# Francesco215/autoregressive_diffusion

Measured on AMD Instinct MI355X. Metric: denoiser-step frames/sec at 1/2/4/8 MI355X; 64-frame Lunar-Lander seq, higher is better.
Workload: dtype bf16; 1 GPU; Lunar-Lander 64-frame seq, gym EDM2 UNet 46.2M (gym_train.py:37-47), 8 seq/GPU (gym_train.py:55 micro_batch_size), step = EDM2Loss fwd + bwd + grad all-reduce + [grad-norm clip +] AdamW + 2 EMA profiles, 3:1 mix of 3-D/2-D steps; global_batch=8, seq_len=64, parallelism=dp1, hip_graph=False

## Files before the change

autoregressive_diffusion_amd/csrc/conv_glds.h:

```cpp
#pragma once
#include <type_traits>
#include "conv_kernels.h"

#include "lds_dma.h"

#ifdef CONV_STAMP
#define CSTAMP_DECL unsigned long long st_t = __builtin_amdgcn_s_memtime(), st_acc[12] = {0, 0, 0, 0, 0, 0, 0, 0, 0, 0, 0, 0};
#define CSTAMP(i) { const unsigned long long n_ = __builtin_amdgcn_s_memtime(); st_acc[i] += n_ - st_t; st_t = n_; }
#define CSTAMP2(c, i, j) { if (c) CSTAMP(i) else CSTAMP(j) }
#else
#define CSTAMP_DECL
#define CSTAMP(i)
#define CSTAMP2(c, i, j)
#endif

template <int NT, int PW, int NW, int MT, int WC = 1>
struct GldsCfg {
  static constexpr int NWP = NW / WC;
  static constexpr int NPOS = 32 * NWP * MT, NTHR = 64 * NW, BN = 32 * NT * WC;
  using P = Patch<PW, NPOS>;
  static constexpr int HW = (PW == 8) ? 12 : PW + 2, HH = P::PH + 2, FT = P::FT;
  static constexpr int HALO = FT * HH * HW;
  static constexpr int SROWS = (HALO + 15) / 16 * 16;
  static constexpr int AROWS = 2 * SROWS, CROWS = HALO, WROWS = 9 * BN;
  static constexpr int BUF = (AROWS + WROWS) * 64;
  static constexpr int EROW = NT * 32 * 2 + 16;
  static constexpr int EPI = NW * 32 * EROW;
  static_assert(PW == 16 || PW == 8, "tile geometries of the LDS-DMA kernel");
  static constexpr int LDS_BYTES = (2 * BUF > EPI) ? 2 * BUF : EPI;
  static_assert(LDS_BYTES <= 160 * 1024, "two staging buffers must fit the 160 KB LDS");
  static constexpr int BUFC = (SROWS + WROWS) * 64;
  static constexpr int RES_EOFF = BUF + 2 * BUFC;
  static constexpr int RES_BYTES = RES_EOFF + 2 * FT * BN * 4 + EPI;
  static_assert(2 * FT * BN * 4 + EPI <= BUF, "the epilogue stages through ONE of the two buffers");
  static_assert((NWP * 2 * HW) % 16 == 0 || MT == 1, "position tiles of a wave must be 16-row aligned apart");
};

template <int NT, int PW, int NW, int MT, int WC = 1, bool CTX = true, bool RES = false>
__global__ __launch_bounds__(64 * NW, (NW >= 8) ? 2 : 1) void conv_glds_kernel(const ConvDev d) {
#if defined(__HIP_DEVICE_COMPILE__)
  using Cfg = GldsCfg<NT, PW, NW, MT, WC>;
  using P = typename Cfg::P;
  constexpr int S = 2, TAPS = 9, CK = 32, KS = CK / 16, HW_ = Cfg::HW, HH_ = Cfg::HH, FT = Cfg::FT, NWP = Cfg::NWP;
  constexpr int NPH = CTX ? 3 : 1;
  constexpr int BN = Cfg::BN, NTHR = Cfg::NTHR, AROWS = Cfg::AROWS, BUF = Cfg::BUF;
  static_assert(!RES || (CTX && FT == 1 && Cfg::RES_BYTES <= 160 * 1024), "resident layout: gated conv, one frame per tile");
  __shared__ __attribute__((aligned(16))) unsigned char smem[RES ? Cfg::RES_BYTES : Cfg::LDS_BYTES];

  const OnirisConvArgs& a = d.a;
  const int tid = threadIdx.x, lane = tid & 63, wave = tid >> 6, r = lane & 31, h = lane >> 5;
  const int wp = wave % NWP, wc = wave / NWP;
  const int H = a.H, W = a.W, T = a.T, Cin = a.Cin, HWp = a.H * a.W;

  const int ntiles = d.ntx * d.nty * d.ntt * a.B * d.ncob;
  int tl, tl_hi, tl_step;
  {
    const int nwg = gridDim.x, xcd = blockIdx.x & 7;
    const int q = ntiles >> 3, rr = ntiles & 7;
    const int lo = (xcd < rr) ? xcd * (q + 1) : rr * (q + 1) + (xcd - rr) * q;
    tl_hi = lo + q + ((xcd < rr) ? 1 : 0);
    tl_step = (nwg - xcd + 7) >> 3;
    tl = lo + (blockIdx.x >> 3);
  }
  if (tl >= tl_hi) return;
  struct Tile { int co0, x0, y0, t0, b; };
  auto decode = [&](int id) __attribute__((always_inline)) {
    Tile t;
    t.co0 = (id % d.ncob) * BN; id /= d.ncob;
    t.x0 = (id % d.ntx) * P::PW; id /= d.ntx;
    t.y0 = (id % d.nty) * P::PH; id /= d.nty;
    t.t0 = (id % d.ntt) * P::FT; id /= d.ntt;
    t.b = id;
    return t;
  };

  int pr = r;
  if constexpr (PW == 16) {
    const bool ga = (r < 4) || (r >= 12 && r < 16) || (r >= 20 && r < 28);
    const int k = ga ? ((r < 4) ? r : (r < 16) ? r - 8 : r - 12) : ((r < 12) ? r - 4 : (r < 20) ? r - 8 : r - 16);
    pr = (ga ? 0 : 16) + k;
  } else {
    const bool ga = (r < 4) || (r >= 12 && r < 16) || (r >= 20 && r < 28);
    const int k = ga ? ((r < 4) ? r : (r < 16) ? r - 8 : r - 12) : ((r < 12) ? r - 4 : (r < 20) ? r - 8 : r - 16);
    pr = ((k >> 3) * 2 + (ga ? 0 : 1)) * 8 + (k & 7);
  }
  int arow[MT];
#pragma unroll
  for (int m = 0; m < MT; ++m) {
    const int p = (wp + NWP * m) * 32 + pr;
    const int ft = p / (P::PH * P::PW), py = (p / P::PW) % P::PH, px = p % P::PW;
    arow[m] = (ft * HH_ + py) * HW_ + px;
  }

  constexpr int TOTA = AROWS * 4, TOTC = Cfg::CROWS * 4, TOTW = Cfg::WROWS * 4;
  constexpr int NIA = (TOTA + NTHR - 1) / NTHR, NIC = (TOTC + NTHR - 1) / NTHR, NIW = (TOTW + NTHR - 1) / NTHR;
  constexpr int OOB = (int)0x80000000;
  const int frame_elems = HWp * Cin;
  int adesc[NIA], wdesc[NIW];
  auto set_adesc = [&](const Tile& t) __attribute__((always_inline)) {
    int tid_ = tid;
    asm volatile("" : "+v"(tid_));
#pragma unroll
    for (int i = 0; i < NIA; ++i) {
      const int e = i * NTHR + tid_;
      const int row = e >> 2, gp = (e & 3) ^ ((row >> 2) & 3);
      const int s = row / Cfg::SROWS, rem = row % Cfg::SROWS;
      const int f_ = rem / (HH_ * HW_), hr = rem % (HH_ * HW_);
      const int y = t.y0 + hr / HW_ - 1, x = t.x0 + hr % HW_ - 1;
      adesc[i] = OOB;
      if (e < TOTA && rem < Cfg::HALO && hr % HW_ < P::PW + 2 && t.t0 + f_ < T && (unsigned)y < (unsigned)H &&
          (unsigned)x < (unsigned)W)
        adesc[i] = ((s * T + f_) * frame_elems + (y * W + x) * Cin + gp * 8) * 2;
    }
  };
#pragma unroll
  for (int i = 0; i < NIW; ++i) {
    const int e = (i * NW + wave) * 64 + lane;
    const int row = e >> 2, gp = (e & 3) ^ ((row >> 2) & 3);
    const int tap = row / BN, co = row % BN;
    wdesc[i] = ((tap * a.CoutP + co) * a.CinP + gp * 8) * 2;
  }
  const int wbytes = TAPS * a.CoutP * a.CinP * 2;
  const i32x4 rs_f = make_rsrc(oniris_fill_rows, 128);
  const i32x4 rs_wo = make_rsrc(a.w_own, wbytes), rs_wc = make_rsrc(CTX ? a.w_ctx : a.w_own, CTX ? 2 * wbytes : wbytes);
  const unsigned lds0 = (unsigned)(size_t)(lds_void_t*)smem;
  const int fillsel = (a.ctx_fill != 0.f) ? 64 : 0;

  auto issue = [&](const Tile& t, int ch, int ph, int bsel) __attribute__((always_inline)) {
    const int c0 = ch * CK;
    const int boff = RES ? ((ph == 0) ? 0 : BUF + (ph - 1) * Cfg::BUFC) : bsel * BUF;
    const int woff = (RES && ph != 0) ? Cfg::SROWS * 64 : AROWS * 64;
    const unsigned dst = __builtin_amdgcn_readfirstlane(lds0 + boff + wave * 1024);
    if (ph == 0) {
      const bf16* xb = (const bf16*)a.x + (size_t)t.b * S * T * frame_elems;
      const i32x4 rs_x = make_rsrc(xb, S * T * frame_elems * 2);
      const int so = (t.t0 * frame_elems + c0) * 2;
#pragma unroll
      for (int i = 0; i < NIA; ++i)
        if ((i * NW + wave) * 64 + lane < TOTA) dma16(rs_x, adesc[i], so, dst + i * NW * 1024);
    } else if constexpr (FT == 1) {
      const int f = t.t0 + ((ph == 1) ? a.coff0 : a.coff1);
      if (f >= 0 && f < a.ctx_T) {
        const bf16* cb_ = (const bf16*)a.ctx + (size_t)t.b * a.ctx_bstride * frame_elems;
        const i32x4 rs_c = make_rsrc(cb_, a.ctx_T * frame_elems * 2);
        const int so = (f * frame_elems + c0) * 2;
#pragma unroll
        for (int i = 0; i < NIC; ++i)
          if ((i * NW + wave) * 64 + lane < TOTC) dma16(rs_c, adesc[i], so, dst + i * NW * 1024);
      } else {
#pragma unroll
        for (int i = 0; i < NIC; ++i)
          if ((i * NW + wave) * 64 + lane < TOTC) dma16(rs_f, (adesc[i] < 0) ? OOB : fillsel, 0, dst + i * NW * 1024);
      }
    } else {
      const int coff = (ph == 1) ? a.coff0 : a.coff1;
      const bf16* cb_ = (const bf16*)a.ctx + (size_t)t.b * a.ctx_bstride * frame_elems;
      const i32x4 rs_c = make_rsrc(cb_, a.ctx_T * frame_elems * 2);
      const int shift = (t.t0 + coff) * frame_elems * 2;
#pragma unroll
      for (int i = 0; i < NIC; ++i) {
        const int e = (i * NW + wave) * 64 + lane;
        if (e < TOTC) {
          const int f = t.t0 + coff + ((e >> 2) % Cfg::SROWS) / (HH_ * HW_);
          if (f >= 0 && f < a.ctx_T) dma16(rs_c, (adesc[i] < 0) ? OOB : adesc[i] + shift, c0 * 2, dst + i * NW * 1024);
          else dma16(rs_f, (adesc[i] < 0) ? OOB : fillsel, 0, dst + i * NW * 1024);
        }
      }
    }
    const int sw = ((t.co0 * a.CinP + c0) + ((ph == 2) ? TAPS * a.CoutP * a.CinP : 0)) * 2;
#ifdef CONV_STAMP
    if (a.big_tile & 64) return;
#endif
    if (ph == 0) {
#pragma unroll
      for (int i = 0; i < NIW; ++i)
        if ((i * NW + wave) * 64 + lane < TOTW) dma16(rs_wo, wdesc[i], sw, dst + woff + i * NW * 1024);
    } else {
#pragma unroll
      for (int i = 0; i < NIW; ++i)
        if ((i * NW + wave) * 64 + lane < TOTW) dma16(rs_wc, wdesc[i], sw, dst + woff + i * NW * 1024);
    }
  };

  const int wa0 = (wc * NT * 32 + r) * 64 + ((h ^ ((r >> 2) & 3)) << 4);
  int xa0[TAPS];
#pragma unroll
  for (int tap = 0; tap < TAPS; ++tap) {
    const int R = arow[0] + (tap / 3) * HW_ + (tap % 3);
    xa0[tap] = R * 64 + ((h ^ ((R >> 2) & 3)) << 4);
  }

  f32x16 acc[S][MT][NT];
  f32x16 accc[MT][NT];

  constexpr int MID_STEP = 4;
  auto mfma_steps = [&](auto own_, int boff, int woff, auto mid) __attribute__((always_inline)) {
    constexpr bool OWN = decltype(own_)::value;
    constexpr int NX = OWN ? S : 1;
    constexpr int NSTEP = TAPS * KS;
    const unsigned char* base = smem + boff;
    const unsigned char* wbase = base + woff;
    bf16x8 wf[2][NT], xf[2][NX][MT];
    auto ld = [&](int fb, int st) __attribute__((always_inline)) {
      const int tap = st / KS, ks = st % KS;
#pragma unroll
      for (int n = 0; n < NT; ++n)
        wf[fb][n] = *(const bf16x8*)(wbase + ((wa0 ^ (ks * 32)) + (tap * BN + n * 32) * 64));
#pragma unroll
      for (int s = 0; s < NX; ++s)
#pragma unroll
        for (int m = 0; m < MT; ++m)
          xf[fb][s][m] = *(const bf16x8*)(base + ((xa0[tap] ^ (ks * 32)) + (s * Cfg::SROWS + m * (NWP * 2 * HW_)) * 64));
    };
    ld(0, 0);
#pragma unroll
    for (int st = 0; st < NSTEP; ++st) {
      mid(st);
      if (st + 1 < NSTEP) ld((st + 1) & 1, st + 1);
#pragma unroll
      for (int m = 0; m < MT; ++m)
#pragma unroll
        for (int n = 0; n < NT; ++n) {
          if constexpr (OWN) {
#pragma unroll
            for (int s = 0; s < S; ++s) acc[s][m][n] = mfma32(wf[st & 1][n], xf[st & 1][s][m], acc[s][m][n]);
          } else {
            accc[m][n] = mfma32(wf[st & 1][n], xf[st & 1][0][m], accc[m][n]);
          }
        }
      if (st + 1 < NSTEP) __builtin_amdgcn_sched_group_barrier(0x100, NT + NX * MT, 0);
      __builtin_amdgcn_sched_group_barrier(0x008, NX * MT * NT, 0);
    }
  };
  auto no_mid = [](int) __attribute__((always_inline)) {};

  constexpr int EROW = Cfg::EROW;
  constexpr int ESC = 2 * FT * BN * 4;
  const int nphase = (Cin / CK) * NPH;
  Tile cur = decode(tl);
  set_adesc(cur);
  int bsel = 0;
  issue(cur, 0, 0, 0);
  if constexpr (RES) { issue(cur, 0, 1, 0); issue(cur, 0, 2, 0); }
  Tile nxt = cur;
  bool more = false;
  int tl_next = tl;
  CSTAMP_DECL
#pragma unroll 1
  for (;;) {
    dma_wait();
    __syncthreads();
    CSTAMP(0)
#pragma unroll
    for (int m = 0; m < MT; ++m)
#pragma unroll
      for (int n = 0; n < NT; ++n) {
#pragma unroll
        for (int i = 0; i < 16; ++i) { acc[0][m][n][i] = 0.f; acc[1][m][n][i] = 0.f; accc[m][n][i] = 0.f; }
      }
    float esc_v = 0.f;
    const int lft = ((wp * 32 + pr) / (P::PH * P::PW)) % FT;
    const bool lvalid = cur.t0 + lft < T;
    const int n0 = (cur.b * S) * T + (lvalid ? cur.t0 + lft : 0), n1 = n0 + T;
    const float cown0 = a.coef_own ? a.coef_own[n0] : 1.f, cown1 = a.coef_own ? a.coef_own[n1] : 1.f;
    const float cctx0 = a.coef_ctx ? a.coef_ctx[n0] : 1.f, cctx1 = a.coef_ctx ? a.coef_ctx[n1] : 1.f;
    if (a.epi == ONIRIS_EPI_EMB_SILU && tid < 2 * FT * BN) {
      const int co = cur.co0 + tid % BN, f_ = (tid / BN) % FT, s_ = tid / (FT * BN);
      if (co < a.Cout && cur.t0 + f_ < T)
        esc_v = ((const float*)a.escale)[(size_t)((cur.b * S + s_) * T + cur.t0 + f_) * (a.escale_pitch ? a.escale_pitch : a.Cout) + co];
    }
    CSTAMP(1)
    if constexpr (!RES) {
#pragma unroll 1
      for (int itp = 0; itp < nphase; ++itp) {
        const int ph = itp % NPH;
        const bool have_next = itp + 1 < nphase;
        const bool early = __builtin_amdgcn_readfirstlane(wave) < NW / 2 || (a.big_tile & 32);
        if (have_next && early) issue(cur, (itp + 1) / NPH, (itp + 1) % NPH, bsel ^ 1);
        auto mid = [&](int st) __attribute__((always_inline)) {
          if (st == MID_STEP && have_next && !early) issue(cur, (itp + 1) / NPH, (itp + 1) % NPH, bsel ^ 1);
        };
        CSTAMP2(ph == 0, 2, 7)
        if (!CTX || ph == 0) mfma_steps(std::true_type{}, bsel * BUF, AROWS * 64, mid);
        else mfma_steps(std::false_type{}, bsel * BUF, AROWS * 64, mid);
#ifdef CONV_STAMP
        asm volatile("" ::"v"(acc[0][0][0]), "v"(acc[1][0][0]), "v"(accc[0][0]), "v"(acc[0][0][NT - 1]), "v"(acc[1][0][NT - 1]), "v"(accc[0][NT - 1]));
#endif
        CSTAMP2(ph == 0, 3, 8)
        dma_wait();
        CSTAMP2(ph == 0, 4, 9)
        __syncthreads();
        CSTAMP2(ph == 0, 5, 10)
        bsel ^= 1;
      }
    }
    unsigned char* stg = smem + (RES ? Cfg::RES_EOFF : (bsel ^ 1) * BUF);
    unsigned char* ep = stg + ESC + wave * 32 * EROW;
    if constexpr (RES) mfma_steps(std::true_type{}, 0, AROWS * 64, no_mid);

    if (a.epi == ONIRIS_EPI_EMB_SILU) {
      if (tid < 2 * FT * BN) *(float*)(stg + tid * 4) = esc_v;
      __syncthreads();
    }
    asm volatile("" ::"v"(cown0), "v"(cown1), "v"(cctx0), "v"(cctx1));
    tl_next = tl + tl_step;
    more = tl_next < tl_hi;
    nxt = cur;
    if constexpr (RES) {
      __syncthreads();
      if (more) { nxt = decode(tl_next); set_adesc(nxt); issue(nxt, 0, 0, 0); }
      mfma_steps(std::false_type{}, BUF, Cfg::SROWS * 64, no_mid);
      __syncthreads();
      if (more) issue(nxt, 0, 1, 0);
      mfma_steps(std::false_type{}, BUF + Cfg::BUFC, Cfg::SROWS * 64, no_mid);
      __syncthreads();
      if (more) issue(nxt, 0, 2, 0);
    } else if (more) {
      nxt = decode(tl_next);
      set_adesc(nxt);
      issue(nxt, 0, 0, bsel);
    }

    bf16* og = (bf16*)a.out;
    bool clip_hit = false;
#pragma unroll
    for (int m = 0; m < MT; ++m) {
      const int ptile = (wp + NWP * m) * 32;
      const int cow = cur.co0 + wc * NT * 32;
      auto flush = [&](bf16* dst, size_t blk) __attribute__((always_inline)) {
        constexpr int PO = NT * 32 / 8;
#pragma unroll
        for (int it = 0; it < 32 * PO / 64; ++it) {
          const int id = it * 64 + lane;
          const int row = id / PO, part = id % PO;
          const int q = ptile + row;
          const int f_ = q / (P::PH * P::PW), yy = (q / P::PW) % P::PH, xx = q % P::PW;
          const size_t px_ = (size_t)(cur.t0 + f_) * HWp + (cur.y0 + yy) * W + (cur.x0 + xx);
          const int co = cow + part * 8;
          if (co < a.Cout && cur.t0 + f_ < T) {
            const u32x4 v_ = *(const u32x4*)(ep + row * EROW + part * 16);
            u32x4* o_ = (u32x4*)(dst + (blk + px_) * a.Cout + co);
            if (d.nt) __builtin_nontemporal_store(v_, o_); else *o_ = v_;
          }
        }
      };
#pragma unroll
      for (int s = 0; s < S; ++s) {
        const float cown = s ? cown1 : cown0, cctx = s ? cctx1 : cctx0;
        const size_t blk = (size_t)(cur.b * S + s) * T * HWp;
        auto raw = [&](int nt, float (&v)[16]) __attribute__((always_inline)) {
#pragma unroll
          for (int i = 0; i < 16; ++i) v[i] = CTX ? __builtin_fmaf(cctx, accc[m][nt][i], cown * acc[s][m][nt][i]) : cown * acc[s][m][nt][i];
        };
        auto put = [&](int nt, const float (&v)[16]) __attribute__((always_inline)) {
#pragma unroll
          for (int g = 0; g < 4; ++g) {
            bf16x4 o;
#pragma unroll
            for (int k = 0; k < 4; ++k) o[k] = f2bf(v[4 * g + k]);
            *(bf16x4*)(ep + pr * EROW + (nt * 32 + 8 * g + 4 * h) * 2) = o;
          }
        };
        float v[16];
        if (a.epi == ONIRIS_EPI_MPSUM) {
          if (a.out2) {
#pragma unroll
            for (int nt = 0; nt < NT; ++nt) { raw(nt, v); put(nt, v); }
            flush((bf16*)a.out2, blk);
          }
          const int p = ptile + pr;
          const size_t obase = (blk + (size_t)(cur.t0 + lft) * HWp + (cur.y0 + (p / P::PW) % P::PH) * W + cur.x0 + p % P::PW) * a.Cout;
#pragma unroll
          for (int nt = 0; nt < NT; ++nt) {
            raw(nt, v);
#pragma unroll
            for (int g = 0; g < 4; ++g) {
              const int co = cow + nt * 32 + 8 * g + 4 * h;
              bf16x4 rv;
#pragma unroll
              for (int k = 0; k < 4; ++k) rv[k] = f2bf(0.f);
              if (co < a.Cout && lvalid) rv = *(const bf16x4*)((const bf16*)a.res + obase + co);
#pragma unroll
              for (int k = 0; k < 4; ++k) {
                float o = a.ta * bf2f(rv[k]) + a.tb * v[4 * g + k];
                if (a.clip > 0.f) {
                  o = fminf(fmaxf(o, -a.clip), a.clip);
                  clip_hit |= !(fabsf(bf2f(f2bf(o))) < a.clip);
                }
                v[4 * g + k] = o;
              }
            }
            put(nt, v);
          }
          flush(og, blk);
        } else {
#pragma unroll
          for (int nt = 0; nt < NT; ++nt) { raw(nt, v); put(nt, v); }
          flush(og, blk);
          if (a.epi == ONIRIS_EPI_EMB_SILU) {
#pragma unroll
            for (int nt = 0; nt < NT; ++nt) {
              raw(nt, v);
#pragma unroll
              for (int g = 0; g < 4; ++g) {
                const float4 ev = *(const float4*)(stg + ((s * FT + lft) * BN + wc * NT * 32 + nt * 32 + 8 * g + 4 * h) * 4);
                const float cvv[4] = {ev.x, ev.y, ev.z, ev.w};
#pragma unroll
                for (int k = 0; k < 4; ++k) {
                  const float z = bf2f(f2bf(v[4 * g + k])) * cvv[k];
                  v[4 * g + k] = z * sigmoid_fast(z) * (1.f / 0.596f);
                }
              }
              put(nt, v);
            }
            flush((bf16*)a.out2, blk);
          }
        }
        if (CTX && a.ctx_out && s == 0) {
#pragma unroll
          for (int nt = 0; nt < NT; ++nt) {
#pragma unroll
            for (int i = 0; i < 16; ++i) v[i] = accc[m][nt][i];
            put(nt, v);
          }
          flush((bf16*)a.ctx_out, (size_t)cur.b * T * HWp);
        }
      }
    }
    if (a.clip_flag && __builtin_amdgcn_ballot_w64(clip_hit) != 0ull) {
      if (lane == 0) atomicOr(a.clip_flag, 1);
    }
    CSTAMP(6)
    if (!more) break;
    cur = nxt;
    tl = tl_next;
  }
#ifdef CONV_STAMP
  if (blockIdx.x == 0 && lane == 0 && a.splitk_ws) {
    unsigned long long* dst = (unsigned long long*)a.splitk_ws + wave * 12;
    for (int i = 0; i < 12; ++i) dst[i] = st_acc[i];
  }
#endif
#endif
}

template <int NT, int PW, int NW, int MT, int WC = 1, bool CTX = true, bool RES = false>
static int launch_conv_glds(const OnirisConvArgs& a, hipStream_t stream) {
  using Cfg = GldsCfg<NT, PW, NW, MT, WC>;
  using P = typename Cfg::P;
  ConvDev d;
  d.a = a;
  d.ksplit = 1; d.reduce = 0;
  d.nt = (long long)a.B * a.S * a.T * a.H * a.W * a.Cout * 2 >= oniris_ew_nt_bytes();
  d.ncob = a.CoutP / Cfg::BN;
  d.ntx = a.W / P::PW; d.nty = a.H / P::PH; d.ntt = cdiv(a.T, P::FT);
  const long long ntiles = (long long)d.ntx * d.nty * d.ntt * a.B * d.ncob;
  if (ntiles <= 0 || ntiles > 0x7fffffffLL) { oniris_set_error("conv_fwd: bad grid %lld", ntiles); return ONIRIS_EINVAL; }
  const int ncu = oniris_persistent_wgs();
  const long long nblk = ntiles < ncu ? ntiles : ncu;
  auto kern = conv_glds_kernel<NT, PW, NW, MT, WC, CTX, RES>;
  oniris_launch_tagged(d.nt ? "nt-stores" : nullptr, kern, dim3((unsigned)nblk), dim3(Cfg::NTHR), stream, d);
  ONIRIS_LAUNCH_CHECK();
  return ONIRIS_OK;
}

static inline bool conv_glds_ok(const OnirisConvArgs& a, int PH, int PW, int BN, bool plain = false) {
  return (plain ? (a.S == 1 && !a.ctx && a.T % 2 == 0) : (a.S == 2 && a.ctx != nullptr)) && a.taps == 9 && a.Cin % 32 == 0 && a.CoutP % BN == 0 && a.H % PH == 0 && a.W % PW == 0 &&
         (a.ctx_fill == 0.f || a.ctx_fill == 1.f) &&
         2LL * a.T * a.H * a.W * a.Cin * 2 < (1LL << 31) && (long long)a.ctx_T * a.H * a.W * a.Cin * 2 < (1LL << 31) &&
         18LL * a.CoutP * a.CinP * 2 < (1LL << 31);
}
```

scratch/conv_stamp.py:

```python
import sys, os, ctypes
sys.path.insert(0, os.path.dirname(os.path.dirname(os.path.abspath(__file__))))
import torch
from autoregressive_diffusion_amd import ops, _lib
from autoregressive_diffusion_amd._lib import lib, check
names = ["tile-top wait", "prologue", "own: dma issue", "mfma", "dma wait", "barrier", "epilogue", "ctx: dma issue", "mfma", "dma wait", "barrier", "-"]
def run(B, T, H, C, Cout, dgrad=False):
    dev = "cuda"
    torch.manual_seed(0)
    p2 = torch.nn.Parameter(torch.randn(Cout, C, 3, 3, device=dev)); p3 = torch.nn.Parameter(torch.randn(Cout, C, 2, 3, 3, device=dev))
    bank = ops.WeightBank(); pw2 = bank.add(p2); pw3 = bank.add(p3); bank.prepare(True)
    N = B * 2 * T
    x = torch.randn(N, H, H, C, device=dev).to(torch.bfloat16)
    c3 = torch.randn(B * T, H, H, C, device=dev).to(torch.bfloat16)
    ca = torch.rand(N, device=dev) + 0.5; cb = torch.rand(N, device=dev) * 0.3
    out = torch.zeros(N, H, H, Cout, device=dev, dtype=torch.bfloat16); y3 = torch.zeros(B * T, H, H, Cout, device=dev, dtype=torch.bfloat16)
    stamps = torch.zeros(96, dtype=torch.int64, device=dev)
    a = _lib.ConvArgs()
    a.x, a.ctx, a.w_own, a.w_ctx, a.out = x.data_ptr(), (c3 if dgrad else x).data_ptr(), pw2.wf.data_ptr(), pw3.wf.data_ptr(), out.data_ptr()
    a.coef_own, a.coef_ctx = ca.data_ptr(), cb.data_ptr()
    a.B, a.S, a.T, a.H, a.W = B, 2, T, H, H
    a.Cin, a.CinP, a.Cout, a.CoutP, a.taps = C, pw2.CinP, Cout, pw2.CoutP, 9
    if dgrad:
        a.ctx_bstride, a.ctx_T, a.coff0, a.coff1, a.ctx_fill = T, T, 2, 1, 0.0
    else:
        a.ctx_bstride, a.ctx_T, a.coff0, a.coff1, a.ctx_fill = 2 * T, T, -2, -1, 1.0
        a.ctx_out = y3.data_ptr()
    a.big_tile = (7 if os.environ.get("NORES") else 4) | (64 if os.environ.get("NOW") else 0)
    a.splitk_ws, a.splitk_ws_bytes = stamps.data_ptr(), 0
    for _ in range(3): check(lib.oniris_conv_fwd(ctypes.byref(a), ops._stream()), "conv")
    torch.cuda.synchronize()
    e0, e1 = torch.cuda.Event(enable_timing=True), torch.cuda.Event(enable_timing=True)
    e0.record()
    for _ in range(10): check(lib.oniris_conv_fwd(ctypes.byref(a), ops._stream()), "conv")
    e1.record(); torch.cuda.synchronize()
    us = e0.elapsed_time(e1) * 100
    fl = 2.0 * N * H * H * Cout * C * 9 * 2
    print(f"{'dgrad' if dgrad else 'fwd'} B={B} T={T} H={H} {C}->{Cout}: {us:.1f} us (stamped build) {fl / us / 1e6:.0f} TFLOP/s")
    s = stamps.view(8, 12).cpu()
    for w in (0, 3, 4, 7):
        tot = int(s[w].sum())
        print(f"  wave {w}: total {tot:7d} | " + " ".join(f"{n} {int(c)}" for n, c in zip(names, s[w]) if n != "-"))
for shp in [(int(os.environ.get("SB", "2")), 64, 32, 64, 64), (int(os.environ.get("SB", "2")), 64, 16, 128, 128)]:
    run(*shp)
```

Baseline: 8532 latent-frames/s.

## Prefetch residual tile via LDS DMA during last MMA phase of MPSUM conv epilogue

```diff
diff --git a/autoregressive_diffusion_amd/csrc/conv_glds.h b/autoregressive_diffusion_amd/csrc/conv_glds.h
--- a/autoregressive_diffusion_amd/csrc/conv_glds.h
+++ b/autoregressive_diffusion_amd/csrc/conv_glds.h
@@ -5,7 +5,7 @@
 #include "lds_dma.h"
 
 #ifdef CONV_STAMP
-#define CSTAMP_DECL unsigned long long st_t = __builtin_amdgcn_s_memtime(), st_acc[12] = {0, 0, 0, 0, 0, 0, 0, 0, 0, 0, 0, 0};
+#define CSTAMP_DECL unsigned long long st_t = __builtin_amdgcn_s_memtime(), st_acc[16] = {0, 0, 0, 0, 0, 0, 0, 0, 0, 0, 0, 0, 0, 0, 0, 0};
 #define CSTAMP(i) { const unsigned long long n_ = __builtin_amdgcn_s_memtime(); st_acc[i] += n_ - st_t; st_t = n_; }
 #define CSTAMP2(c, i, j) { if (c) CSTAMP(i) else CSTAMP(j) }
 #else
@@ -33,6 +33,8 @@
   static constexpr int RES_EOFF = BUF + 2 * BUFC;
   static constexpr int RES_BYTES = RES_EOFF + 2 * FT * BN * 4 + EPI;
   static_assert(2 * FT * BN * 4 + EPI <= BUF, "the epilogue stages through ONE of the two buffers");
+  static constexpr int RTILE = 32 * NT * 64;
+  static_assert(2 * FT * BN * 4 + 2 * NW * RTILE <= BUF, "both slots' residual tiles must fit ONE of the two buffers");
   static_assert((NWP * 2 * HW) % 16 == 0 || MT == 1, "position tiles of a wave must be 16-row aligned apart");
 };
 
@@ -179,6 +181,33 @@
 #pragma unroll
       for (int i = 0; i < NIW; ++i)
         if ((i * NW + wave) * 64 + lane < TOTW) dma16(rs_wc, wdesc[i], sw, dst + woff + i * NW * 1024);
+    }
+  };
+
+  constexpr int PO = NT * 32 / 8, RROW = NT * 64, RTILE = Cfg::RTILE, NPR = RTILE / 1024;
+  auto rsw = [](int row) __attribute__((always_inline)) { return (NT == 2) ? (row & 7) : ((row >> 2) & 3); };
+  auto issue_res = [&](const Tile& t, int bsel_) __attribute__((always_inline)) {
+    constexpr int RPP = 64 / PO;
+    static_assert(MT == 1 && (P::PW % RPP == 0 || RPP % P::PW == 0) && RPP % 8 == 0, "a piece is half a tile row or whole tile rows");
+    int lane_ = lane;
+    asm volatile("" : "+v"(lane_));
+    const int ll = lane_ / PO, co = t.co0 + wc * NT * 32 + ((lane_ % PO) ^ rsw(ll)) * 8;
+    const int voff = (co < a.Cout) ? (((ll / P::PW) * W + ll % P::PW) * a.Cout + co) * 2 : OOB;
+    const int nvf = (T - t.t0 < FT) ? T - t.t0 : FT;
+    const unsigned dst = __builtin_amdgcn_readfirstlane(lds0 + bsel_ * BUF + 2 * FT * BN * 4 + wave * RTILE);
+    const int wp_ = __builtin_amdgcn_readfirstlane(wp);
+#pragma unroll
+    for (int s = 0; s < S; ++s) {
+      const long long blk = (long long)(t.b * S + s) * T * HWp;
+      const long long org = blk + (long long)t.t0 * HWp + t.y0 * W + t.x0;
+      const long long left = (blk + (long long)(t.t0 + nvf) * HWp - org) * a.Cout * 2;
+      const i32x4 rs_r = make_rsrc((const bf16*)a.res + org * a.Cout, (int)(left < 0x7fffffffLL ? left : 0x7fffffffLL));
+#pragma unroll
+      for (int it = 0; it < NPR; ++it) {
+        const int q = wp_ * 32 + it * RPP;
+        const int so = (q / (P::PH * P::PW) * HWp + (q / P::PW) % P::PH * W + q % P::PW) * a.Cout * 2;
+        dma16(rs_r, voff, so, dst + s * NW * RTILE + it * 1024);
+      }
     }
   };
 
@@ -276,9 +305,14 @@
         const int ph = itp % NPH;
         const bool have_next = itp + 1 < nphase;
         const bool early = __builtin_amdgcn_readfirstlane(wave) < NW / 2 || (a.big_tile & 32);
-        if (have_next && early) issue(cur, (itp + 1) / NPH, (itp + 1) % NPH, bsel ^ 1);
+        const bool res_dma = !have_next && a.epi == ONIRIS_EPI_MPSUM;
+        auto feed = [&]() __attribute__((always_inline)) {
+          if (have_next) issue(cur, (itp + 1) / NPH, (itp + 1) % NPH, bsel ^ 1);
+          else if (res_dma) issue_res(cur, bsel ^ 1);
+        };
+        if (early) feed();
         auto mid = [&](int st) __attribute__((always_inline)) {
-          if (st == MID_STEP && have_next && !early) issue(cur, (itp + 1) / NPH, (itp + 1) % NPH, bsel ^ 1);
+          if (st == MID_STEP && !early) feed();
         };
         CSTAMP2(ph == 0, 2, 7)
         if (!CTX || ph == 0) mfma_steps(std::true_type{}, bsel * BUF, AROWS * 64, mid);
@@ -294,7 +328,7 @@
         bsel ^= 1;
       }
     }
-    unsigned char* stg = smem + (RES ? Cfg::RES_EOFF : (bsel ^ 1) * BUF);
+    unsigned char* stg = smem + (RES ? Cfg::RES_EOFF : bsel * BUF);
     unsigned char* ep = stg + ESC + wave * 32 * EROW;
     if constexpr (RES) mfma_steps(std::true_type{}, 0, AROWS * 64, no_mid);
 
@@ -318,8 +352,9 @@
     } else if (more) {
       nxt = decode(tl_next);
       set_adesc(nxt);
-      issue(nxt, 0, 0, bsel);
-    }
+      issue(nxt, 0, 0, bsel ^ 1);
+    }
+    if constexpr (!RES) bsel ^= 1;
 
     bf16* og = (bf16*)a.out;
     bool clip_hit = false;
@@ -327,20 +362,39 @@
     for (int m = 0; m < MT; ++m) {
       const int ptile = (wp + NWP * m) * 32;
       const int cow = cur.co0 + wc * NT * 32;
-      auto flush = [&](bf16* dst, size_t blk) __attribute__((always_inline)) {
-        constexpr int PO = NT * 32 / 8;
-#pragma unroll
-        for (int it = 0; it < 32 * PO / 64; ++it) {
-          const int id = it * 64 + lane;
-          const int row = id / PO, part = id % PO;
-          const int q = ptile + row;
-          const int f_ = q / (P::PH * P::PW), yy = (q / P::PW) % P::PH, xx = q % P::PW;
-          const size_t px_ = (size_t)(cur.t0 + f_) * HWp + (cur.y0 + yy) * W + (cur.x0 + xx);
-          const int co = cow + part * 8;
-          if (co < a.Cout && cur.t0 + f_ < T) {
-            const u32x4 v_ = *(const u32x4*)(ep + row * EROW + part * 16);
-            u32x4* o_ = (u32x4*)(dst + (blk + px_) * a.Cout + co);
-            if (d.nt) __builtin_nontemporal_store(v_, o_); else *o_ = v_;
+      int lane_e = lane, pr_e = pr, h_e = h;
+      asm volatile("" : "+v"(lane_e), "+v"(pr_e), "+v"(h_e));
+      constexpr int RPP = 64 / PO;
+      const int ll_e = lane_e / PO, co_e = cow + ((lane_e % PO) ^ rsw(ll_e)) * 8;
+      const unsigned off_e = (((ll_e / P::PW) * W + ll_e % P::PW) * a.Cout + co_e) * 2;
+      const bool ok_e = co_e < a.Cout && cur.t0 + ptile / (P::PH * P::PW) < T;
+      auto flush = [&](auto lin_, const unsigned char* tile, bf16* dst, size_t blk) __attribute__((always_inline)) {
+        if constexpr (decltype(lin_)::value) {
+          const char* base = (const char*)(dst + (blk + (size_t)cur.t0 * HWp + cur.y0 * W + cur.x0) * a.Cout);
+#pragma unroll
+          for (int it = 0; it < NPR; ++it) {
+            const int q = __builtin_amdgcn_readfirstlane(ptile) + it * RPP;
+            const int so = (q / (P::PH * P::PW) * HWp + (q / P::PW) % P::PH * W + q % P::PW) * a.Cout * 2;
+            if (ok_e) {
+              const u32x4 v_ = *(const u32x4*)(tile + it * 1024 + lane_e * 16);
+              u32x4* o_ = (u32x4*)(base + so + off_e);
+              if (d.nt) __builtin_nontemporal_store(v_, o_); else *o_ = v_;
+            }
+          }
+        } else {
+#pragma unroll
+          for (int it = 0; it < 32 * PO / 64; ++it) {
+            const int id = it * 64 + lane;
+            const int row = id / PO, part = id % PO;
+            const int q = ptile + row;
+            const int f_ = q / (P::PH * P::PW), yy = (q / P::PW) % P::PH, xx = q % P::PW;
+            const size_t px_ = (size_t)(cur.t0 + f_) * HWp + (cur.y0 + yy) * W + (cur.x0 + xx);
+            const int co = cow + part * 8;
+            if (co < a.Cout && cur.t0 + f_ < T) {
+              const u32x4 v_ = *(const u32x4*)(tile + row * EROW + part * 16);
+              u32x4* o_ = (u32x4*)(dst + (blk + px_) * a.Cout + co);
+              if (d.nt) __builtin_nontemporal_store(v_, o_); else *o_ = v_;
+            }
           }
         }
       };
@@ -352,34 +406,30 @@
 #pragma unroll
           for (int i = 0; i < 16; ++i) v[i] = CTX ? __builtin_fmaf(cctx, accc[m][nt][i], cown * acc[s][m][nt][i]) : cown * acc[s][m][nt][i];
         };
-        auto put = [&](int nt, const float (&v)[16]) __attribute__((always_inline)) {
+        auto rt_at = [&](unsigned char* tile, int nt, int g) __attribute__((always_inline)) {
+          return tile + pr_e * RROW + (((nt * 4 + g) ^ rsw(pr_e)) << 4) + h_e * 8;
+        };
+        auto put = [&](auto lin_, unsigned char* tile, int nt, const float (&v)[16]) __attribute__((always_inline)) {
 #pragma unroll
           for (int g = 0; g < 4; ++g) {
             bf16x4 o;
 #pragma unroll
             for (int k = 0; k < 4; ++k) o[k] = f2bf(v[4 * g + k]);
-            *(bf16x4*)(ep + pr * EROW + (nt * 32 + 8 * g + 4 * h) * 2) = o;
+            if constexpr (decltype(lin_)::value) *(bf16x4*)rt_at(tile, nt, g) = o;
+            else *(bf16x4*)(tile + pr * EROW + (nt * 32 + 8 * g + 4 * h) * 2) = o;
           }
         };
+        constexpr std::integral_constant<bool, !RES> LIN{};
         float v[16];
-        if (a.epi == ONIRIS_EPI_MPSUM) {
-          if (a.out2) {
-#pragma unroll
-            for (int nt = 0; nt < NT; ++nt) { raw(nt, v); put(nt, v); }
-            flush((bf16*)a.out2, blk);
-          }
-          const int p = ptile + pr;
-          const size_t obase = (blk + (size_t)(cur.t0 + lft) * HWp + (cur.y0 + (p / P::PW) % P::PH) * W + cur.x0 + p % P::PW) * a.Cout;
+        unsigned char* rt = RES ? ep : stg + ESC + (s * NW + wave) * RTILE;
+        if (!RES && a.epi == ONIRIS_EPI_MPSUM) {
+          CSTAMP(6)
 #pragma unroll
           for (int nt = 0; nt < NT; ++nt) {
             raw(nt, v);
 #pragma unroll
             for (int g = 0; g < 4; ++g) {
-              const int co = cow + nt * 32 + 8 * g + 4 * h;
-              bf16x4 rv;
-#pragma unroll
-              for (int k = 0; k < 4; ++k) rv[k] = f2bf(0.f);
-              if (co < a.Cout && lvalid) rv = *(const bf16x4*)((const bf16*)a.res + obase + co);
+              const bf16x4 rv = *(const bf16x4*)rt_at(rt, nt, g);
 #pragma unroll
               for (int k = 0; k < 4; ++k) {
                 float o = a.ta * bf2f(rv[k]) + a.tb * v[4 * g + k];
@@ -390,13 +440,52 @@
                 v[4 * g + k] = o;
               }
             }
-            put(nt, v);
-          }
-          flush(og, blk);
+            put(LIN, rt, nt, v);
+          }
+          CSTAMP(12)
+          flush(LIN, rt, og, blk);
+          CSTAMP(13)
+          if (a.out2) {
+#pragma unroll
+            for (int nt = 0; nt < NT; ++nt) { raw(nt, v); put(LIN, rt, nt, v); }
+            flush(LIN, rt, (bf16*)a.out2, blk);
+          }
+          CSTAMP(14)
+        } else if (RES && a.epi == ONIRIS_EPI_MPSUM) {
+          if (a.out2) {
+#pragma unroll
+            for (int nt = 0; nt < NT; ++nt) { raw(nt, v); put(LIN, rt, nt, v); }
+            flush(LIN, rt, (bf16*)a.out2, blk);
+          }
+          const int p = ptile + pr;
+          const size_t obase = (blk + (size_t)(cur.t0 + lft) * HWp + (cur.y0 + (p / P::PW) % P::PH) * W + cur.x0 + p % P::PW) * a.Cout;
+#pragma unroll
+          for (int nt = 0; nt < NT; ++nt) {
+            raw(nt, v);
+#pragma unroll
+            for (int g = 0; g < 4; ++g) {
+              const int co = cow + nt * 32 + 8 * g + 4 * h;
+              bf16x4 rv;
+#pragma unroll
+              for (int k = 0; k < 4; ++k) rv[k] = f2bf(0.f);
+              if (co < a.Cout && lvalid) rv = *(const bf16x4*)((const bf16*)a.res + obase + co);
+#pragma unroll
+              for (int k = 0; k < 4; ++k) {
+                float o = a.ta * bf2f(rv[k]) + a.tb * v[4 * g + k];
+                if (a.clip > 0.f) {
+                  o = fminf(fmaxf(o, -a.clip), a.clip);
+                  clip_hit |= !(fabsf(bf2f(f2bf(o))) < a.clip);
+                }
+                v[4 * g + k] = o;
+              }
+            }
+            put(LIN, rt, nt, v);
+          }
+          flush(LIN, rt, og, blk);
         } else {
 #pragma unroll
-          for (int nt = 0; nt < NT; ++nt) { raw(nt, v); put(nt, v); }
-          flush(og, blk);
+          for (int nt = 0; nt < NT; ++nt) { raw(nt, v); put(LIN, rt, nt, v); }
+          flush(LIN, rt, og, blk);
           if (a.epi == ONIRIS_EPI_EMB_SILU) {
 #pragma unroll
             for (int nt = 0; nt < NT; ++nt) {
@@ -411,19 +500,21 @@
                   v[4 * g + k] = z * sigmoid_fast(z) * (1.f / 0.596f);
                 }
               }
-              put(nt, v);
+              put(LIN, rt, nt, v);
             }
-            flush((bf16*)a.out2, blk);
+            flush(LIN, rt, (bf16*)a.out2, blk);
           }
         }
+        CSTAMP(6)
         if (CTX && a.ctx_out && s == 0) {
 #pragma unroll
           for (int nt = 0; nt < NT; ++nt) {
 #pragma unroll
             for (int i = 0; i < 16; ++i) v[i] = accc[m][nt][i];
-            put(nt, v);
-          }
-          flush((bf16*)a.ctx_out, (size_t)cur.b * T * HWp);
+            put(LIN, rt, nt, v);
+          }
+          flush(LIN, rt, (bf16*)a.ctx_out, (size_t)cur.b * T * HWp);
+          CSTAMP(15)
         }
       }
     }
@@ -437,8 +528,8 @@
   }
 #ifdef CONV_STAMP
   if (blockIdx.x == 0 && lane == 0 && a.splitk_ws) {
-    unsigned long long* dst = (unsigned long long*)a.splitk_ws + wave * 12;
-    for (int i = 0; i < 12; ++i) dst[i] = st_acc[i];
+    unsigned long long* dst = (unsigned long long*)a.splitk_ws + wave * 16;
+    for (int i = 0; i < 16; ++i) dst[i] = st_acc[i];
   }
 #endif
 #endif
@@ -468,5 +559,6 @@
   return (plain ? (a.S == 1 && !a.ctx && a.T % 2 == 0) : (a.S == 2 && a.ctx != nullptr)) && a.taps == 9 && a.Cin % 32 == 0 && a.CoutP % BN == 0 && a.H % PH == 0 && a.W % PW == 0 &&
          (a.ctx_fill == 0.f || a.ctx_fill == 1.f) &&
          2LL * a.T * a.H * a.W * a.Cin * 2 < (1LL << 31) && (long long)a.ctx_T * a.H * a.W * a.Cin * 2 < (1LL << 31) &&
-         18LL * a.CoutP * a.CinP * 2 < (1LL << 31);
+         18LL * a.CoutP * a.CinP * 2 < (1LL << 31) &&
+         2LL * a.H * a.W * a.Cout * 2 < (1LL << 31);
 }
diff --git a/scratch/conv_stamp.py b/scratch/conv_stamp.py
--- a/scratch/conv_stamp.py
+++ b/scratch/conv_stamp.py
@@ -3,7 +3,8 @@
 import torch
 from autoregressive_diffusion_amd import ops, _lib
 from autoregressive_diffusion_amd._lib import lib, check
-names = ["tile-top wait", "prologue", "own: dma issue", "mfma", "dma wait", "barrier", "epilogue", "ctx: dma issue", "mfma", "dma wait", "barrier", "-"]
+names = ["tile-top wait", "prologue", "own: dma issue", "mfma", "dma wait", "barrier", "epilogue (rest)", "ctx: dma issue", "mfma", "dma wait", "barrier",
+         "res: first-value wait", "res math+put", "flush out", "out2 round", "ctx_out round"]
 def run(B, T, H, C, Cout, dgrad=False):
     dev = "cuda"
     torch.manual_seed(0)
@@ -14,7 +15,8 @@
     c3 = torch.randn(B * T, H, H, C, device=dev).to(torch.bfloat16)
     ca = torch.rand(N, device=dev) + 0.5; cb = torch.rand(N, device=dev) * 0.3
     out = torch.zeros(N, H, H, Cout, device=dev, dtype=torch.bfloat16); y3 = torch.zeros(B * T, H, H, Cout, device=dev, dtype=torch.bfloat16)
-    stamps = torch.zeros(96, dtype=torch.int64, device=dev)
+    stamps = torch.zeros(128, dtype=torch.int64, device=dev)
+    res = torch.randn(N, H, H, Cout, device=dev).to(torch.bfloat16); out2 = torch.zeros_like(out)
     a = _lib.ConvArgs()
     a.x, a.ctx, a.w_own, a.w_ctx, a.out = x.data_ptr(), (c3 if dgrad else x).data_ptr(), pw2.wf.data_ptr(), pw3.wf.data_ptr(), out.data_ptr()
     a.coef_own, a.coef_ctx = ca.data_ptr(), cb.data_ptr()
@@ -25,6 +27,8 @@
     else:
         a.ctx_bstride, a.ctx_T, a.coff0, a.coff1, a.ctx_fill = 2 * T, T, -2, -1, 1.0
         a.ctx_out = y3.data_ptr()
+    if os.environ.get("EPI") == "2" and not dgrad:
+        a.epi, a.res, a.out2, a.ta, a.tb, a.clip = _lib.EPI_MPSUM, res.data_ptr(), out2.data_ptr(), 0.7, 0.5, 256.0
     a.big_tile = (7 if os.environ.get("NORES") else 4) | (64 if os.environ.get("NOW") else 0)
     a.splitk_ws, a.splitk_ws_bytes = stamps.data_ptr(), 0
     for _ in range(3): check(lib.oniris_conv_fwd(ctypes.byref(a), ops._stream()), "conv")
@@ -36,9 +40,10 @@
     us = e0.elapsed_time(e1) * 100
     fl = 2.0 * N * H * H * Cout * C * 9 * 2
     print(f"{'dgrad' if dgrad else 'fwd'} B={B} T={T} H={H} {C}->{Cout}: {us:.1f} us (stamped build) {fl / us / 1e6:.0f} TFLOP/s")
-    s = stamps.view(8, 12).cpu()
+    s = stamps.view(8, 16).cpu()
     for w in (0, 3, 4, 7):
         tot = int(s[w].sum())
-        print(f"  wave {w}: total {tot:7d} | " + " ".join(f"{n} {int(c)}" for n, c in zip(names, s[w]) if n != "-"))
-for shp in [(int(os.environ.get("SB", "2")), 64, 32, 64, 64), (int(os.environ.get("SB", "2")), 64, 16, 128, 128)]:
+        print(f"  wave {w}: total {tot:7d} | " + " ".join(f"{n} {int(c)}" for n, c in zip(names, s[w])))
+SB = int(os.environ.get("SB", "2"))
+for shp in [(SB, 64, 32, 64, 64), (SB, 64, 16, 128, 128)] + ([(SB, 64, 8, 256, 256)] if os.environ.get("SHAPES") == "fwd" else []):
     run(*shp)
```

After: 8466 latent-frames/s. Within noise of the previous version (-0.8%).
